# howird/humanoid

Measured on NVIDIA B200. Metric: env_steps_per_sec, higher is better.
Workload: dtype f32

## Files before the change

humanoid_b200/csrc/phc_kernels.cu:

```cuda
#include <algorithm>
#include <atomic>
#include <cfloat>
#include <cstdint>
#include <cstdio>
#include <cstdlib>
#include <cstring>
#include <new>

#include <cuda_bf16.h>
#include <cuda_runtime.h>

#include "../../include/phc_b200.h"
#include "phc_math.cuh"

namespace phc {

constexpr int J24 = PHC_NUM_BODIES;
constexpr int SELF_DIM = PHC_SELF_OBS_DIM;
constexpr int TASK_DIM = PHC_TASK_OBS_DIM;

static thread_local int g_last_cuda_error = 0;

static inline int cuda_fail(cudaError_t e) {
  g_last_cuda_error = (int)e;
// ... 889 lines not shown

constexpr int ROW13 = J24 * 13;
constexpr int FRAME_FLOATS = J24 * 13;
constexpr int FRAME_F4 = FRAME_FLOATS / 4;
constexpr int STAGE_FLOATS = SELF_DIM + TASK_DIM;

constexpr int EP_SUM_COLS = 12;

struct StepParams {
  LibDev L;
  PhcBodyState body;
  int16_t* progress;
  int16_t* progress_mirror;
  const float* start;
  const float* start_off;
  const float* goff;
  const int64_t* ids;
  const float* term_dist;
  uint32_t reset_mask;
  int use_mean, early, advance, T;
  float dt;
  PhcRewardSpec rwd;
  float* obs;
  int64_t obs_stride;
  float* rew;
  float* raw;
  int64_t raw_stride;
  uint8_t* reset;
  uint8_t* term;
  double* moments;
  int moment_buckets;
  int multi_prefetch;
  int moments_bulk;
  uint8_t *ep_terminals, *ep_truncations, *ep_masks;
  float* ep_returns;
  int32_t* ep_lengths;
  double* ep_sums;
  int ep_buckets, ep_raw_cols;
  float* mpjpe;
  float* obs_norm;
  int64_t obs_norm_stride;
  const float* norm_mean;
  const float* norm_var;
  float norm_eps, norm_clip;
  int norm_bf16;
  const float* dof_force;
  int64_t dof_force_stride;
  const float* dof_vel;
  int64_t dof_vel_stride, dof_vel_estride;
  float power_coef;
  int power_col;
  int64_t n;
  int first_wave_blocks;
  int spec_fault;
  unsigned long long* trace;
  const uint8_t* env_mask;
  int obs_only;
  int aos;
  int obs_vec2;
  float* rew_out;
  uint8_t* reset_out;
  uint8_t* term_out;
  float* ref_dof_pos;
  int64_t ref_dof_pos_stride;
  ObsFlags of;
  int selfw;
  int reset_on;
  ResetTargets rw;
  unsigned* tile_counter;
};

__host__ __device__ __forceinline__ bool default_obs_flags(const ObsFlags& f) { return f.hcol && f.local_root && f.upright; }

__device__ __forceinline__ void write_ref_dof_pos(const StepParams& p, int64_t env, int b, int64_t f0, int64_t f1, float bl) {
  if (b < 1) return;
  const Quat lr = quat_slerp(ld4v(p.L.lrs + (f0 * J24 + b) * 4), ld4v(p.L.lrs + (f1 * J24 + b) * 4), bl);
  st3(p.ref_dof_pos + env * p.ref_dof_pos_stride + (b - 1) * 3, quat_exp_map(lr));
}

__device__ __forceinline__ float norm_clamp(float y, float clip) { return y < -clip ? -clip : (y > clip ? clip : y); }
__device__ __forceinline__ void norm_column(const float* means, const float* vars, float eps, int64_t col, float& mean,
                                            float& sd, float& r) {
  mean = means[col];
  const float v = vars[col] + eps;
  sd = v >= FLT_MIN && v <= FLT_MAX ? sqrt_faithful(v) : sqrtf(v);
  r = rcp_approx(sd);
}
__device__ __forceinline__ void norm_column(const StepParams& p, int64_t col, float& mean, float& sd, float& r) {
  norm_column(p.norm_mean, p.norm_var, p.norm_eps, col, mean, sd, r);
}
__device__ __forceinline__ float norm_value(float x, float mean, float sd, float r, float clip) {
  const float a = x - mean;
  const float y = div_faithful(a, sd, r);
  return norm_clamp(y != y ? a * r : y, clip);
}

__device__ __forceinline__ float power_partial(const StepParams& p, int64_t env, int b) {
  if (b == 0) return 0.0f;
  const float* f = p.dof_force + env * p.dof_force_stride + (b - 1) * 3;
  const float* v = p.dof_vel + env * p.dof_vel_stride + (int64_t)(b - 1) * 3 * p.dof_vel_estride;
  return (fabsf(__ldcg(f) * __ldcg(v)) + fabsf(__ldcg(f + 1) * __ldcg(v + p.dof_vel_estride))) +
         fabsf(__ldcg(f + 2) * __ldcg(v + 2 * p.dof_vel_estride));
}
__device__ __forceinline__ float power_reward(const StepParams& p, const float* row24, int prog) {
  const float r = (-p.power_coef) * row_sum24(row24);
  return prog <= 3 ? 0.0f : r;
// ... 446 lines not shown
  static_assert(EPB * J24 == 96, "three warps, one role each");
  const int w = threadIdx.x >> 5, b = threadIdx.x & 31;
  const bool act = b < J24;
  const float len = S.meta_len[f], mdt = S.meta_mdt[f];
  const int nf = S.meta_nf[f];
  const int64_t st = S.meta_st[f];
  const float t = reset_start_time(p.rw, env, len);
  RefBody own;
  if (act) {
    int64_t f0, f1;
    float bl;
    reset_query_frames32(w == 1 ? 1 : 0, p.dt, t, len, nf, mdt, st, f0, f1, bl);
    if (w < 2) {
      const bool A = w == 0;
      own = blend_ref3(p.L.packed + f0 * FRAME_FLOATS, p.L.packed + f1 * FRAME_FLOATS, bl, A ? S.goff[f][0] : 0.0f,
                       A ? S.goff[f][1] : 0.0f, A ? S.goff[f][2] : 0.0f, b);
      if (A) {
        reset_store_body(p.rw, env, b, t, own.pos, own.rot, own.vel, own.ang, false);
        put13(S.sim + f * ROW13 + b * 13, own.pos, own.rot, own.vel, own.ang);
        if (b == 0) {
          if (p.progress_mirror) p.progress_mirror[env] = 0;
          const Heading h0 = heading_quat_inv(heading_source(own.rot, p.of.upright));
          S.nroot[f][0] = own.pos.x, S.nroot[f][1] = own.pos.y, S.nroot[f][2] = own.pos.z;
          S.nroot[f][3] = h0.z, S.nroot[f][4] = h0.w;
        }
      }
    } else {
      reset_store_dof(p.L, p.rw, env, b, f0, f1, bl);
      if (p.ref_dof_pos && b >= 1) {
        int64_t g0, g1;
        float gl;
        reset_query_frames32(1, p.dt, t, len, nf, mdt, st, g0, g1, gl);
        const Quat lr = quat_slerp(ld4v(p.L.lrs + (g0 * J24 + b) * 4), ld4v(p.L.lrs + (g1 * J24 + b) * 4), gl);
        st3(p.ref_dof_pos + env * p.ref_dof_pos_stride + (b - 1) * 3, quat_exp_map(lr));
      }
    }
  }
  __syncthreads();
  if (!act || w == 2) return;
  const int SW = DEF ? SELF_DIM : p.selfw;
  const Vec3 root_pos = {S.nroot[f][0], S.nroot[f][1], S.nroot[f][2]};
  const Heading hi = {S.nroot[f][3], S.nroot[f][4]};
  const HeadingRot hr = heading_rot(hi);
  float* row = S.frames + f * (SW + TASK_DIM);
  if (w == 0) {
    emit_self_obs<DEF>(row, p.of, b, root_pos, hi, hr, own.pos, own.rot, own.vel, own.ang);
  } else {
    const float* d = S.sim + f * ROW13 + b * 13;
    emit_task_obs<DEF>(row + SW, b, hi, hr, root_pos, Vec3{d[0], d[1], d[2]}, Quat{d[3], d[4], d[5], d[6]},
                       Vec3{d[7], d[8], d[9]}, Vec3{d[10], d[11], d[12]}, own);
  }
}

template <int EPB, int MINB, bool NORM = false, bool EP = false, bool RESET = false, bool DEF = true>
__global__ void __launch_bounds__(EPB* J24, MINB) step_fast_kernel(const __grid_constant__ StepParams p) {
  extern __shared__ __align__(16) unsigned char smem_raw[];
  FastSmem<EPB>& S = *reinterpret_cast<FastSmem<EPB>*>(smem_raw);
  constexpr int NT = EPB * J24;
  static_assert(4 * EPB <= 32, "reductions run on one warp");
  static_assert(!NORM || DEF, "the normaliser epilogue is laid out for the default 934-float rows");
  const int tid = threadIdx.x;
  const int64_t env0 = (int64_t)blockIdx.x * EPB;
  const int nvalid = p.n <= env0 ? 0 : (int)((p.n - env0) < EPB ? (p.n - env0) : EPB);
  PHC_STAMP(0);

  if (p.first_wave_blocks > 0) asm volatile("griddepcontrol.launch_dependents;\n" ::: "memory");
  const bool speculate = blockIdx.x < (unsigned)p.first_wave_blocks;
  if (tid < 32) {
    static_assert(EPB == 4, "phase 0 maps 8 lanes to each of 4 envs");
    if (tid == 0) mbar_init(&S.bar, 1);
    __syncwarp();
    const int le = tid >> 3, j = tid & 7;
    const bool act = le < nvalid;
    const bool lead = act && j == 0;
    const int64_t env = env0 + (act ? le : 0);
    const int adv = p.advance ? 1 : 0;
    float* fr = S.frames + le * (4 * FRAME_FLOATS);
    int64_t sid = -1, st = 0;
    int nf = 2, sprog = 0;
    float len = 1.0f, mdt = 1.0f, sstart = 0.0f, ssoff = 0.0f;
    int c_f0 = 0, c_f1 = 0;
    float c_bl = 0.0f, c_t = 0.0f;
    if (speculate && act && j < 3) {
      sid = p.ids[env];
      sprog = (int)p.progress[env];
      sstart = p.start[env];
      ssoff = p.start_off[env];
      if (p.spec_fault) {
        if (p.spec_fault & 1) sprog -= 1;
        if (p.spec_fault & 2) sstart += 1.0f / 30.0f;
        if (p.spec_fault & 4) sprog -= 2;
        if (p.spec_fault & 8) sid += 1;
      }
      const int64_t c = sid < 0 ? 0 : (sid >= p.L.M ? p.L.M - 1 : sid);
      len = p.L.len[c];
      nf = (int)p.L.nf[c];
      mdt = p.L.mdt[c];
      st = p.L.starts[c];
      c_t = (float)(int16_t)(sprog + adv + j) * p.dt + sstart + ssoff;
      calc_frame_blend32(c_t, len, nf, mdt, c_f0, c_f1, c_bl);
    }
    const int hi1 = __shfl_sync(0xffffffffu, c_f1, (tid & ~7) + 1);
    const int hi2 = __shfl_sync(0xffffffffu, c_f1, (tid & ~7) + 2);
    const int s_lo = c_f0;
    const bool all3 = hi2 - s_lo <= 3 && hi2 >= hi1;
    const int s_hi = all3 ? hi2 : hi1;
    const bool spec = speculate && lead && s_hi - s_lo <= 3 && s_hi >= s_lo;
    if (spec) {
      const uint32_t bytes = (uint32_t)(s_hi - s_lo + 1) * (uint32_t)(FRAME_FLOATS * 4);
      mbar_expect_tx(&S.bar, bytes);
      bulk_g2s(fr, p.L.packed + (st + s_lo) * FRAME_FLOATS, bytes, &S.bar);
    }
    const bool block_sim = p.body.pos.stride_env == ROW13;
    if (speculate && lead && (block_sim ? le == 0 : true)) {
      const uint32_t bytes = (block_sim ? (uint32_t)nvalid : 1u) * (uint32_t)(ROW13 * 4);
      asm volatile("cp.async.bulk.prefetch.L2.global [%0], %1;\n" ::"l"(p.body.pos.ptr + env * p.body.pos.stride_env),
                   "r"(bytes)
                   : "memory");
    }
    asm volatile("griddepcontrol.wait;\n" ::: "memory");
    if (p.first_wave_blocks <= 0) asm volatile("griddepcontrol.launch_dependents;\n" ::: "memory");
    PHC_STAMP(2);
    int prog_in = 0;
    bool ok = false;
    float start = 0.0f, soff = 0.0f, g0 = 0.0f, g1 = 0.0f, g2 = 0.0f;
    int64_t id = 0;
    if (lead) {
      prog_in = (int)__ldcg(p.progress + env);
      id = __ldcg(p.ids + env);
      start = __ldcg(p.start + env);
      soff = __ldcg(p.start_off + env);
      if (p.goff) {
        g0 = __ldcg(p.goff + env * 3 + 0);
        g1 = __ldcg(p.goff + env * 3 + 1);
        g2 = __ldcg(p.goff + env * 3 + 2);
      }
      if (block_sim ? le == 0 : true) {
        const uint32_t bytes = (block_sim ? (uint32_t)nvalid : 1u) * (uint32_t)(ROW13 * 4);
        mbar_expect_tx(&S.bar, bytes);
        bulk_g2s(S.sim + le * ROW13, p.body.pos.ptr + env * p.body.pos.stride_env, bytes, &S.bar);
      }
      const int dd = prog_in - sprog;
      ok = speculate && id == sid && __float_as_uint(start) == __float_as_uint(sstart) &&
           __float_as_uint(soff) == __float_as_uint(ssoff) && (dd == 0 || (dd == 1 && all3));
    }
    const int d = (prog_in - sprog) & 1;
    const int src0 = (tid & ~7) + d, src1 = src0 + 1;
    int a_f0 = __shfl_sync(0xffffffffu, c_f0, src0), a_f1 = __shfl_sync(0xffffffffu, c_f1, src0);
    int b_f0 = __shfl_sync(0xffffffffu, c_f0, src1), b_f1 = __shfl_sync(0xffffffffu, c_f1, src1);
    float a_bl = __shfl_sync(0xffffffffu, c_bl, src0), b_bl = __shfl_sync(0xffffffffu, c_bl, src1);
    float a_t = __shfl_sync(0xffffffffu, c_t, src0);
    const bool redo = lead && spec && !ok;
    const unsigned any_redo = __ballot_sync(0xffffffffu, redo);
    if (any_redo) {
      if (tid == 0) mbar_arrive(&S.bar);
      mbar_wait(&S.bar, 0);
    }
    if (lead) {
      int prog = prog_in;
      if (p.advance) prog = (int)(int16_t)(prog + 1);
      if (!ok) {
        len = p.L.len[id];
        nf = (int)p.L.nf[id];
        mdt = p.L.mdt[id];
        st = p.L.starts[id];
        a_t = (float)(int16_t)prog * p.dt + start + soff;
        calc_frame_blend32(a_t, len, nf, mdt, a_f0, a_f1, a_bl);
        const float t1 = (float)(int16_t)(prog + 1) * p.dt + start + soff;
        calc_frame_blend32(t1, len, nf, mdt, b_f0, b_f1, b_bl);
      }
      S.bl[0][le] = a_bl;
      S.bl[1][le] = b_bl;
      S.prog[le] = prog;
      S.pass[le] = a_t >= len;
      S.fallen[le] = 0;
      if (p.advance) {
        p.progress[env] = (int16_t)prog;
        if (p.progress_mirror) p.progress_mirror[env] = (int16_t)prog;
      }
      S.goff[le][0] = g0;
      S.goff[le][1] = g1;
      S.goff[le][2] = g2;
      if (RESET) {
        S.meta_len[le] = len, S.meta_mdt[le] = mdt, S.meta_nf[le] = nf, S.meta_st[le] = st;
      }
      if (p.ref_dof_pos) S.row1[0][le] = st + b_f0, S.row1[1][le] = st + b_f1;
      if (ok && spec) {
        S.slot[0][0][le] = a_f0 - s_lo;
        S.slot[0][1][le] = a_f1 - s_lo;
        S.slot[1][0][le] = b_f0 - s_lo;
        S.slot[1][1][le] = b_f1 - s_lo;
      } else {
        const float* tab = p.L.packed + st * FRAME_FLOATS;
        const int lo = a_f0 < b_f0 ? a_f0 : b_f0;
        int hi = a_f1 > b_f1 ? a_f1 : b_f1;
        hi = hi > a_f0 ? hi : a_f0;
        hi = hi > b_f0 ? hi : b_f0;
        if (hi - lo <= 3) {
          S.slot[0][0][le] = a_f0 - lo;
          S.slot[0][1][le] = a_f1 - lo;
          S.slot[1][0][le] = b_f0 - lo;
          S.slot[1][1][le] = b_f1 - lo;
          const uint32_t bytes = (uint32_t)(hi - lo + 1) * (uint32_t)(FRAME_FLOATS * 4);
          mbar_expect_tx(&S.bar, bytes);
          bulk_g2s(fr, tab + (int64_t)lo * FRAME_FLOATS, bytes, &S.bar);
        } else {
          S.slot[0][0][le] = 0;
          S.slot[0][1][le] = a_f1 - a_f0;
          S.slot[1][0][le] = 2;
          S.slot[1][1][le] = 2 + (b_f1 - b_f0);
          const uint32_t ba = (uint32_t)(a_f1 - a_f0 + 1) * (uint32_t)(FRAME_FLOATS * 4);
          const uint32_t bb = (uint32_t)(b_f1 - b_f0 + 1) * (uint32_t)(FRAME_FLOATS * 4);
          mbar_expect_tx(&S.bar, ba + bb);
          bulk_g2s(fr, tab + (int64_t)a_f0 * FRAME_FLOATS, ba, &S.bar);
          bulk_g2s(fr + 2 * FRAME_FLOATS, tab + (int64_t)b_f0 * FRAME_FLOATS, bb, &S.bar);
        }
      }
    }
    __syncwarp();
    if (tid == 0) {
      S.parity = any_redo ? 1 : 0;
      mbar_arrive(&S.bar);
    }
    PHC_STAMP(1);
  } else {
    asm volatile("griddepcontrol.wait;\n" ::: "memory");
    if (tid >= 32 && tid < 32 + nvalid) {
      const int le = tid - 32;
      const float* rq = p.body.pos.ptr + (env0 + le) * p.body.pos.stride_env + 3;
      const Quat rq4 = Quat{__ldcg(rq), __ldcg(rq + 1), __ldcg(rq + 2), __ldcg(rq + 3)};
      const Heading h0 = heading_quat_inv(DEF ? rq4 : heading_source(rq4, p.of.upright));
      S.hz[le] = h0.z;
      S.hw[le] = h0.w;
    }
  }
  __syncthreads();
  mbar_wait(&S.bar, (uint32_t)S.parity);
  PHC_STAMP(3);

  const int e = tid / J24, b = tid % J24;
  const bool valid = e < nvalid;
  Vec3 pos, vel, ang;
  Quat rot;
  RefBody r1;
  if (valid) {
    const float* d = S.sim + e * ROW13 + b * 13;
    pos = {d[0], d[1], d[2]};
    rot = {d[3], d[4], d[5], d[6]};
    vel = {d[7], d[8], d[9]};
    ang = {d[10], d[11], d[12]};
    const float* fr = S.frames + e * (4 * FRAME_FLOATS);
    {
      const RefBody r0 = blend_ref2(fr + S.slot[0][0][e] * FRAME_FLOATS, fr + S.slot[0][1][e] * FRAME_FLOATS,
                                    S.bl[0][e], S.goff[e], b);
      float sp, sr, sv, sa;
      reward_partials(pos, rot, vel, ang, r0, sp, sr, sv, sa);
      S.part[0][e][b] = sp;
      S.part[1][e][b] = sr;
      S.part[2][e][b] = sv;
      S.part[3][e][b] = sa;
      const float dist = norm3(pos - r0.pos);
      S.part[4][e][b] = dist;
      if (!p.use_mean && (p.reset_mask >> b & 1u) && dist > p.term_dist[b]) S.fallen[e] = 1;
      if (p.dof_force) S.part[5][e][b] = power_partial(p, env0 + e, b);
    }
    r1 = blend_ref2(fr + S.slot[1][0][e] * FRAME_FLOATS, fr + S.slot[1][1][e] * FRAME_FLOATS, S.bl[1][e], S.goff[e], b);
  }
  PHC_STAMP(4);
  __syncthreads();

  bool my_rst = false;
  int rst_mask = 0;
  if constexpr (RESET) {
    if (p.reset_on) {
      if (p.use_mean) {
        if (tid < nvalid) {
          float sel[J24];
          int m = 0;
#pragma unroll
          for (int j = 0; j < J24; ++j)
            if (p.reset_mask >> j & 1u) sel[m++] = S.part[4][tid][j];
          const int first = __ffs(p.reset_mask) - 1;
          bool fallen = p.early && m > 0 && (aten_row_sum(sel, m) / (float)m) > p.term_dist[first < 0 ? 0 : first];
          fallen = fallen && (S.prog[tid] > 1);
          S.rst[tid] = (S.pass[tid] || fallen) ? 1 : 0;
        }
        __syncthreads();
      }
#pragma unroll
      for (int i = 0; i < EPB; ++i) {
        int r = 0;
        if (i < nvalid) r = p.use_mean ? S.rst[i] : ((S.pass[i] || (p.early && S.fallen[i] && S.prog[i] > 1)) ? 1 : 0);
        rst_mask |= r << i;
        if (i == e) my_rst = valid && r;
      }
#pragma unroll
      for (int i = 0; i < EPB; ++i)
        if (rst_mask >> i & 1) reset_prefetch<EPB>(p, S, i, env0 + i);
    }
  }

  const int SW = DEF ? SELF_DIM : p.selfw;
  const int RW = SW + TASK_DIM;
  if (valid && !(RESET && my_rst)) {
    const Vec3 root_pos = {S.sim[e * ROW13 + 0], S.sim[e * ROW13 + 1], S.sim[e * ROW13 + 2]};
    const Heading hi = {S.hz[e], S.hw[e]};
    const HeadingRot hr = heading_rot(hi);
    float* row = S.frames + e * RW;
    emit_self_obs<DEF>(row, p.of, b, root_pos, hi, hr, pos, rot, vel, ang);
    emit_task_obs<DEF>(row + SW, b, hi, hr, root_pos, pos, rot, vel, ang, r1);
  }
  if constexpr (RESET) {
    if (rst_mask) {
#pragma unroll 1
      for (int i = 0; i < EPB; ++i)
        if (rst_mask >> i & 1) reset_in_step<EPB, DEF>(p, S, i, env0 + i);
    }
  }
  fence_proxy_async();
  PHC_STAMP(5);
  __syncthreads();
  PHC_STAMP(6);

  const uint32_t out_bytes = (uint32_t)nvalid * (uint32_t)(RW * 4);
  const bool bulk_ok = (out_bytes & 15u) == 0;
  if (bulk_ok) {
    if (tid == NT - 1 && out_bytes) bulk_s2g(p.obs + env0 * RW, S.frames, out_bytes);
  } else if (DEF || ((nvalid * RW) & 1) == 0) {
    float2* dst = reinterpret_cast<float2*>(p.obs + env0 * RW);
    const float2* src = reinterpret_cast<const float2*>(S.frames);
    for (int i = tid; i < nvalid * RW / 2; i += NT) dst[i] = src[i];
  } else {
    for (int i = tid; i < nvalid * RW; i += NT) p.obs[env0 * RW + i] = S.frames[i];
  }
  if (p.moments) {
    double* mom = p.moments + (int64_t)(blockIdx.x % p.moment_buckets) * 2 * RW;
    if (p.moments_bulk) {
      constexpr int CH = 624;
      static_assert(CH * 8 <= (int)sizeof(S.sim) && CH * 8 <= (int)sizeof(S.frames) - EPB * STAGE_FLOATS * 4, "regions");
      double* regA = reinterpret_cast<double*>(S.sim);
      double* regB = reinterpret_cast<double*>(S.frames + EPB * RW);
      const int total = 2 * RW;
      for (int c0 = 0, r = 0; c0 < total; c0 += CH, ++r) {
        double* reg = (r & 1) ? regB : regA;
        const int cnt = total - c0 < CH ? total - c0 : CH;
        if (r >= 2) {
          if (tid == 0) bulk_wait_read_all_but_one();
          __syncthreads();
        }
        for (int i = tid; i < cnt; i += NT) {
          const int g = c0 + i;
          const bool sq = g >= RW;
          const int col = sq ? g - RW : g;
          double acc = 0.0;
          for (int ee = 0; ee < nvalid; ++ee) {
            const double x = (double)S.frames[ee * RW + col];
            acc += sq ? x * x : x;
          }
          reg[i] = acc;
        }
        fence_proxy_async();
        __syncthreads();
        if (tid == 0) bulk_reduce_add_f64(mom + c0, reg, (uint32_t)cnt * 8u);
      }
      if (NORM && p.obs_norm) {
        if (tid == 0) bulk_wait_read();
        __syncthreads();
      }
    } else {
      for (int c = tid; c < RW; c += NT) {
        double s1 = 0.0, s2 = 0.0;
        for (int ee = 0; ee < nvalid; ++ee) {
          const double x = (double)S.frames[ee * RW + c];
          s1 += x;
          s2 += x * x;
        }
        atomicAdd(mom + c, s1);
        atomicAdd(mom + RW + c, s2);
      }
    }
  }
  if (p.ref_dof_pos && valid && !(RESET && my_rst))
    write_ref_dof_pos(p, env0 + e, b, S.row1[0][e], S.row1[1][e], S.bl[1][e]);
  const bool norm_inplace = NORM && p.obs_norm && bulk_ok && !p.norm_bf16;
  if (norm_inplace) {
    if (tid == NT - 1) bulk_wait_read();
    __syncthreads();
    float2* st = reinterpret_cast<float2*>(S.frames);
    for (int c2 = tid; c2 < STAGE_FLOATS / 2; c2 += NT) {
      float m0, sd0, r0, m1, sd1, r1;
      norm_column(p, 2 * c2, m0, sd0, r0);
      norm_column(p, 2 * c2 + 1, m1, sd1, r1);
      for (int ee = 0; ee < nvalid; ++ee) {
        const float2 x = st[ee * (STAGE_FLOATS / 2) + c2];
        st[ee * (STAGE_FLOATS / 2) + c2] =
            make_float2(norm_value(x.x, m0, sd0, r0, p.norm_clip), norm_value(x.y, m1, sd1, r1, p.norm_clip));
      }
    }
    fence_proxy_async();
    __syncthreads();
    if (tid == NT - 1) bulk_s2g(p.obs_norm + env0 * STAGE_FLOATS, S.frames, out_bytes);
  }
  constexpr int NORM16_SPLIT = 932;
  static_assert(EPB != 4 || (NORM16_SPLIT * 4 <= (int)sizeof(S.sim) && (EPB * STAGE_FLOATS / 2 - NORM16_SPLIT) * 4 <=
                                 (int)sizeof(S.frames) - EPB * STAGE_FLOATS * 4), "bf16 staging fits the dead regions");
  const bool norm16_staged =
      NORM && p.obs_norm && bulk_ok && p.norm_bf16 && nvalid == EPB && EPB == 4 && ((uintptr_t)p.obs_norm & 15) == 0;
  if (norm16_staged) {
    __nv_bfloat162* pa = reinterpret_cast<__nv_bfloat162*>(S.sim);
    __nv_bfloat162* pb = reinterpret_cast<__nv_bfloat162*>(S.frames + EPB * STAGE_FLOATS);
    const float2* src = reinterpret_cast<const float2*>(S.frames);
    for (int c2 = tid; c2 < STAGE_FLOATS / 2; c2 += NT) {
      float m0, sd0, r0, m1, sd1, r1;
      norm_column(p, 2 * c2, m0, sd0, r0);
      norm_column(p, 2 * c2 + 1, m1, sd1, r1);
#pragma unroll
      for (int ee = 0; ee < EPB; ++ee) {
        const int i = ee * (STAGE_FLOATS / 2) + c2;
        const float2 x = src[i];
        const __nv_bfloat162 y = __floats2bfloat162_rn(norm_value(x.x, m0, sd0, r0, p.norm_clip),
                                                       norm_value(x.y, m1, sd1, r1, p.norm_clip));
        if (i < NORM16_SPLIT) pa[i] = y;
        else pb[i - NORM16_SPLIT] = y;
      }
    }
    fence_proxy_async();
    __syncthreads();
    if (tid == NT - 1) {
      __nv_bfloat162* dst = reinterpret_cast<__nv_bfloat162*>(p.obs_norm) + env0 * (STAGE_FLOATS / 2);
      bulk_s2g(dst, pa, NORM16_SPLIT * 4);
      bulk_s2g(dst + NORM16_SPLIT, pb, (EPB * STAGE_FLOATS / 2 - NORM16_SPLIT) * 4);
    }
  }
  if (tid < 32) {
    const int le = tid >> 2, k = tid & 3;
    const bool act = le < nvalid && tid < 4 * EPB;
    float term_k = 0.0f;
    float ep_ret = 0.0f;
    int32_t ep_len = 0;
    if constexpr (EP) {
      if (p.ep_returns && act && k == 0) {
        ep_ret = p.ep_returns[env0 + le];
        ep_len = p.ep_lengths[env0 + le];
      }
    }
    if (act) {
      const float kk = k == 0 ? p.rwd.k_pos : k == 1 ? p.rwd.k_rot : k == 2 ? p.rwd.k_vel : p.rwd.k_ang_vel;
      term_k = expf((-kk) * (row_sum24(&S.part[k][le][0]) / 24.0f));
      p.raw[(env0 + le) * p.raw_stride + k] = term_k;
    }
    const int base = tid & ~3;
    const float t0 = __shfl_sync(0xffffffffu, term_k, base), t1 = __shfl_sync(0xffffffffu, term_k, base + 1);
    const float t2 = __shfl_sync(0xffffffffu, term_k, base + 2), t3 = __shfl_sync(0xffffffffu, term_k, base + 3);
    float r = 0.0f, pr = 0.0f;
    int flags = 0;
    if (act && k == 0) {
      r = p.rwd.w_pos * t0 + p.rwd.w_rot * t1 + p.rwd.w_vel * t2 + p.rwd.w_ang_vel * t3;
      if (p.dof_force) {
        pr = power_reward(p, &S.part[5][le][0], S.prog[le]);
        r += pr;
        p.raw[(env0 + le) * p.raw_stride + p.power_col] = pr;
      }
      p.rew[env0 + le] = r;
      if (p.rew_out) p.rew_out[env0 + le] = r;
    }
    if (act && k == 1) {
      bool fallen = false;
      if (p.early) {
        if (p.use_mean) {
          float sel[J24];
          int m = 0;
#pragma unroll
          for (int j = 0; j < J24; ++j)
            if (p.reset_mask >> j & 1u) sel[m++] = S.part[4][le][j];
          const int first = __ffs(p.reset_mask) - 1;
          fallen = m > 0 && (aten_row_sum(sel, m) / (float)m) > p.term_dist[first < 0 ? 0 : first];
        } else {
          fallen = S.fallen[le] != 0;
        }
        fallen = fallen && (S.prog[le] > 1);
      }
      const bool rs = S.pass[le] || fallen;
      const bool cleared = RESET && p.reset_on;
      p.term[env0 + le] = (fallen && !cleared) ? 1 : 0;
      p.reset[env0 + le] = (rs && !cleared) ? 1 : 0;
      if (p.term_out) p.term_out[env0 + le] = fallen ? 1 : 0;
      if (p.reset_out) p.reset_out[env0 + le] = rs ? 1 : 0;
      flags = (rs ? 1 : 0) | (fallen ? 2 : 0);
    }
    if (act && k == 2 && p.mpjpe) p.mpjpe[env0 + le] = row_sum24(&S.part[4][le][0]) / 24.0f;
    if constexpr (EP) if (p.ep_returns) {
      flags = __shfl_sync(0xffffffffu, flags, base + 1);
      float v[EP_SUM_COLS];
#pragma unroll
      for (int i = 0; i < EP_SUM_COLS; ++i) v[i] = 0.0f;
      if (act && k == 0) {
        const int64_t e = env0 + le;
        const bool rs = flags & 1, tm = (flags & 2) != 0, tr = rs && !tm;
        p.ep_terminals[e] = tm ? 1 : 0;
        p.ep_truncations[e] = tr ? 1 : 0;
        p.ep_masks[e] = tr ? 0 : 1;
        float ret = ep_ret;
        int32_t len = ep_len;
        if (rs) {
          v[0] = 1.0f;
          v[1] = ret;
          v[2] = (float)len;
          v[3] = tr ? 1.0f : 0.0f;
          ret = 0.0f;
          len = 0;
        }
        p.ep_returns[e] = ret + r;
        p.ep_lengths[e] = len + 1;
        v[4] = t0, v[5] = t1, v[6] = t2, v[7] = t3;
        if (p.dof_force) {
#pragma unroll
          for (int i = 8; i < EP_SUM_COLS; ++i)
            if (i == 4 + p.power_col) v[i] = pr;
        }
      }
      float mine = 0.0f;
#pragma unroll
      for (int i = 0; i < EP_SUM_COLS; ++i) {
        v[i] += __shfl_xor_sync(0xffffffffu, v[i], 4);
        v[i] += __shfl_xor_sync(0xffffffffu, v[i], 8);
        const float tot = __shfl_sync(0xffffffffu, v[i], 0);
        if (tid == i) mine = tot;
      }
      if (tid < 4 + p.ep_raw_cols && mine != 0.0f)
        atomicAdd(p.ep_sums + (int64_t)(blockIdx.x % p.ep_buckets) * EP_SUM_COLS + tid, (double)mine);
    }
  }

  if (NORM && p.obs_norm && !norm_inplace && !norm16_staged) {
    float2* dst = reinterpret_cast<float2*>(p.obs_norm + env0 * STAGE_FLOATS);
    __nv_bfloat162* dst16 = reinterpret_cast<__nv_bfloat162*>(p.obs_norm) + env0 * (STAGE_FLOATS / 2);
    const float2* src = reinterpret_cast<const float2*>(S.frames);
    for (int c2 = tid; c2 < STAGE_FLOATS / 2; c2 += NT) {
      float m0, sd0, r0, m1, sd1, r1;
      norm_column(p, 2 * c2, m0, sd0, r0);
      norm_column(p, 2 * c2 + 1, m1, sd1, r1);
      for (int ee = 0; ee < nvalid; ++ee) {
        const float2 x = src[ee * (STAGE_FLOATS / 2) + c2];
        const float y0 = norm_value(x.x, m0, sd0, r0, p.norm_clip), y1 = norm_value(x.y, m1, sd1, r1, p.norm_clip);
        if (p.norm_bf16) dst16[ee * (STAGE_FLOATS / 2) + c2] = __floats2bfloat162_rn(y0, y1);
        else dst[ee * (STAGE_FLOATS / 2) + c2] = make_float2(y0, y1);
      }
    }
  }
  if (bulk_ok && tid == NT - 1) bulk_wait_read();
  if (p.moments && p.moments_bulk && tid == 0) bulk_wait_read();
  PHC_STAMP(7);
}

constexpr int PS_STAGES = 2;
constexpr int PS_EPB = 4;
constexpr int PS_CONSUMERS = PS_EPB * J24;
constexpr int PS_THREADS = PS_CONSUMERS + 32;

template <int SLOTS>
struct PersistStage {
  float sim[PS_EPB * ROW13];
  float frames[PS_EPB * SLOTS * FRAME_FLOATS];
  float part[6][PS_EPB][J24];
  float bl[2][PS_EPB];
  int slot[2][2][PS_EPB];
  int64_t far[PS_EPB];
  float goff[PS_EPB][4];
  float hz[PS_EPB], hw[PS_EPB];
  int prog[PS_EPB], pass[PS_EPB], fallen[PS_EPB];
  int tile;
  int pad_[3];
  static_assert(SLOTS * FRAME_FLOATS >= STAGE_FLOATS, "the obs stage aliases the frame buffer");
};
template <int SLOTS>
struct PersistSmem {
  PersistStage<SLOTS> st[PS_STAGES];
  unsigned long long full[PS_STAGES], empty[PS_STAGES];
};
static_assert(sizeof(PersistStage<3>) % 16 == 0 && sizeof(PersistStage<4>) % 16 == 0,
              "stages keep the 16-byte alignment of the TMA destinations");

__device__ __forceinline__ void consumer_sync() { asm volatile("bar.sync 1, %0;" ::"r"(PS_CONSUMERS) : "memory"); }

template <int SLOTS, int BLOCKS_PER_SM, bool MOM = false>
__global__ void __launch_bounds__(PS_THREADS, BLOCKS_PER_SM) step_persist_kernel(const __grid_constant__ StepParams p) {
  extern __shared__ __align__(16) unsigned char smem_raw[];
  PersistSmem<SLOTS>& M = *reinterpret_cast<PersistSmem<SLOTS>*>(smem_raw);
  using Stage = PersistStage<SLOTS>;
  const int tid = threadIdx.x;
  const int num_tiles = (int)((p.n + PS_EPB - 1) / PS_EPB);
  if (tid == 0) {
#pragma unroll
    for (int s = 0; s < PS_STAGES; ++s) {
      mbar_init(&M.full[s], 1);
      mbar_init(&M.empty[s], MOM ? PS_CONSUMERS / 32 : 1);
    }
  }
  __syncthreads();

  if (tid >= PS_CONSUMERS) {
    const int lane = tid - PS_CONSUMERS;
    const int le = lane >> 3, j = lane & 7;
    asm volatile("griddepcontrol.launch_dependents;\n" ::: "memory");
// ... 1468 lines not shown
  p.raw_stride = a->reward_raw_stride;
  p.reset = a->reset_buf;
  p.term = a->terminate_buf;
  p.moments = a->obs_moments;
  p.moment_buckets = a->obs_moments_buckets > 1 ? a->obs_moments_buckets : 1;
  p.moments_bulk = 0;
  {
    static int mp = -1;
    if (mp < 0) {
      const char* w = getenv("PHC_MULTI_PREFETCH");
      mp = (w && w[0] == '0') ? 0 : 1;
    }
    p.multi_prefetch = mp;
  }
  p.ep_terminals = a->ep_terminals;
  p.ep_truncations = a->ep_truncations;
  p.ep_masks = a->ep_masks;
  p.ep_returns = a->ep_returns;
  p.ep_lengths = a->ep_lengths;
  p.ep_sums = a->ep_sums;
  p.ep_buckets = a->ep_buckets;
  p.ep_raw_cols = a->ep_raw_cols;
  if (a->ep_returns) {
    if (!a->ep_terminals || !a->ep_truncations || !a->ep_masks || !a->ep_lengths || !a->ep_sums) return PHC_ERR_NULL;
    if (a->ep_buckets < 1 || a->ep_buckets > 4096 || a->ep_raw_cols < 0 || a->ep_raw_cols > EP_SUM_COLS - 4) return PHC_ERR_SHAPE;
  }
  if (a->obs_moments_buckets < 0 || a->obs_moments_buckets > 4096) return PHC_ERR_SHAPE;
  p.mpjpe = a->mpjpe;
  p.obs_norm = a->obs_norm;
  p.obs_norm_stride = a->obs_norm_stride;
  p.norm_mean = a->norm_mean;
  p.norm_var = a->norm_var;
  p.norm_eps = a->norm_epsilon;
  p.norm_clip = a->norm_clip;
  p.norm_bf16 = (a->flags & PHC_STEP_OBS_NORM_BF16) ? 1 : 0;
  if (a->obs_norm) {
    if (!a->norm_mean || !a->norm_var) return PHC_ERR_NULL;
    if (a->obs_norm_stride < W || !(a->norm_clip > 0.0f)) return PHC_ERR_SHAPE;
  }
  p.dof_force = a->dof_force;
  p.dof_force_stride = a->dof_force_stride;
  p.dof_vel = a->dof_vel;
  p.dof_vel_stride = a->dof_vel_stride;
  p.dof_vel_estride = a->dof_vel_elem_stride;
  p.power_coef = a->rew_power_coef;
  p.power_col = a->power_col;
  if (a->dof_force) {
    if (!a->dof_vel) return PHC_ERR_NULL;
    if (a->power_col < 4 || a->power_col >= a->reward_raw_stride || a->dof_force_stride < 69 ||
        a->dof_vel_elem_stride < 1)
      return PHC_ERR_SHAPE;
  }
  p.first_wave_blocks = 0;
  p.spec_fault = g_spec_fault;
  p.env_mask = nullptr;
  p.obs_only = 0;
  {
    const int64_t nw = (n + 3) / 4 * 3;
    if (g_trace && (g_trace_launch + 1) * nw <= g_trace_capacity) {
      p.trace = g_trace + g_trace_launch * nw * 8;
      ++g_trace_launch;
    } else {
      p.trace = nullptr;
    }
  }
  p.n = n;
  const PhcBodyState& s = a->body;
  p.aos = s.rot.ptr == s.pos.ptr + 3 && s.vel.ptr == s.pos.ptr + 7 && s.ang_vel.ptr == s.pos.ptr + 10 &&
          s.pos.stride_body == 13 && s.rot.stride_body == 13 && s.vel.stride_body == 13 &&
          s.ang_vel.stride_body == 13 && s.rot.stride_env == s.pos.stride_env &&
          s.vel.stride_env == s.pos.stride_env && s.ang_vel.stride_env == s.pos.stride_env &&
          ((uintptr_t)s.pos.ptr & 15) == 0 && (s.pos.stride_env % 4) == 0 && s.pos.stride_env >= ROW13;
  p.obs_vec2 = ((uintptr_t)a->obs_buf & 7) == 0 && (a->obs_stride % 2) == 0;
  return PHC_OK;
}

static int g_force_generic = -1;
static int g_fast_epb = -1;
static int g_pdl = -1;

static void init_options() {
  if (g_force_generic < 0) {
    const char* v = getenv("PHC_STEP_GENERIC");
    g_force_generic = (v && v[0] == '1') ? 1 : 0;
  }
  if (g_fast_epb < 0) {
    const char* w = getenv("PHC_STEP_EPB");
    g_fast_epb = (w && w[0] == '8') ? 8 : 4;
  }
  if (g_pdl < 0) {
    const char* w = getenv("PHC_STEP_PDL");
    g_pdl = (w && w[0] == '0') ? 0 : 1;
  }
  if (g_moments_bulk < 0) {
    const char* w = getenv("PHC_MOMENTS_BULK");
    g_moments_bulk = (w && w[0] == '1') ? 1 : 0;
  }
  if (g_persist < 0) {
    const char* w = getenv("PHC_STEP_PERSIST");
    g_persist = (w && w[0] >= '0' && w[0] <= '3') ? w[0] - '0' : 1;
    g_persist_pdl = g_pdl;
    const char* m = getenv("PHC_STEP_PERSIST_MIN");
    if (m && atoll(m) > 0) g_persist_min = atoll(m);
  }
}

// ... 83 lines not shown
                                     ((uintptr_t)p.obs_norm & (p.norm_bf16 ? 3 : 15)) == 0));
  static bool attr_gen[64] = {};
  static int first_wave[64] = {};
  static bool attr_persist[3][64] = {};
  static int sm_count[64] = {};
  const bool persist = fast && def && g_persist != 0 &&
                       (g_persist >= 2 || p.n >= (p.moments ? g_persist_min_moments : g_persist_min)) && !p.obs_norm &&
                       !p.ep_returns && !p.reset_on && !p.ref_dof_pos && !p.trace && lib->tile_counters &&
                       !(args->flags & PHC_STEP_MAPPED_HOST_IO);
  if (persist) {
    if (!sm_count[dev]) PHC_CUDA(cudaDeviceGetAttribute(&sm_count[dev], cudaDevAttrMultiProcessorCount, dev));
    const bool mom = p.moments != nullptr;
    const bool four = !mom && g_persist == 3;
    const int which = mom ? 2 : four ? 1 : 0;
    auto kern = mom ? step_persist_kernel<3, 4, true> : four ? step_persist_kernel<4, 4> : step_persist_kernel<3, 5>;
    const size_t smem = four ? sizeof(PersistSmem<4>) : sizeof(PersistSmem<3>);
    if (!attr_persist[which][dev]) {
      PHC_CUDA(cudaFuncSetAttribute(kern, cudaFuncAttributeMaxDynamicSharedMemorySize, (int)smem));
      attr_persist[which][dev] = true;
    }
    if (lib->unspeculated_steps > 0) --lib->unspeculated_steps;
    p.tile_counter = lib->tile_counters + 2 * (lib->tile_seq.fetch_add(1u, std::memory_order_relaxed) % TILE_SLOTS);
    const int64_t tiles = (p.n + PS_EPB - 1) / PS_EPB;
    const int64_t resident = (int64_t)sm_count[dev] * (four || mom ? 4 : 5);
    cudaLaunchConfig_t cfg{};
    cfg.gridDim = dim3((unsigned)(tiles < resident ? tiles : resident));
    cfg.blockDim = dim3(PS_THREADS);
    cfg.dynamicSmemBytes = smem;
    cfg.stream = stream;
    cudaLaunchAttribute at[1];
    at[0].id = cudaLaunchAttributeProgrammaticStreamSerialization;
    at[0].val.programmaticStreamSerializationAllowed = 1;
    cfg.attrs = at;
    cfg.numAttrs = g_persist_pdl ? 1 : 0;
    PHC_CUDA(cudaLaunchKernelEx(&cfg, kern, p));
    return launch_status();
  }
  bool reset_after = false;
  if (fast) {
    if (!first_wave[dev]) {
      int sms = 0, per_sm = 0;
      PHC_CUDA(cudaDeviceGetAttribute(&sms, cudaDevAttrMultiProcessorCount, dev));
      PHC_CUDA(cudaFuncSetAttribute(step_fast_kernel<4, 8>, cudaFuncAttributeMaxDynamicSharedMemorySize,
                                    (int)sizeof(FastSmem<4>)));
      PHC_CUDA(cudaOccupancyMaxActiveBlocksPerMultiprocessor(&per_sm, step_fast_kernel<4, 8>, 4 * J24,
                                                             sizeof(FastSmem<4>)));
      first_wave[dev] = sms * (per_sm > 0 ? per_sm : 1);
    }
    p.first_wave_blocks = (g_pdl && !(args->flags & PHC_STEP_MAPPED_HOST_IO)) ? first_wave[dev] : 0;
    if (lib->unspeculated_steps > 0) {
      p.first_wave_blocks = 0;
      --lib->unspeculated_steps;
    }
    static bool attr[7][64] = {};
    const bool pdl = g_pdl != 0;
    constexpr size_t SM = sizeof(FastSmem<4>);
    p.moments_bulk = (p.moments && g_moments_bulk && ((uintptr_t)p.moments & 15) == 0) ? 1 : 0;
    const bool in_kernel = p.reset_on && p.rw.state_init <= PHC_STATE_INIT_RANDOM;
    reset_after = p.reset_on && !in_kernel;
    StepParams pk = p;
    if (reset_after) pk.reset_on = 0;
    if (!def) rc = launch_step(step_fast_kernel<4, 8, false, true, true, false>, SM, 4, pk, stream, &attr[6][dev], pdl);
    else if (in_kernel) {
      if (p.obs_norm) rc = launch_step(step_fast_kernel<4, 8, true, true, true>, SM, 4, pk, stream, &attr[5][dev], pdl);
      else rc = launch_step(step_fast_kernel<4, 8, false, true, true>, SM, 4, pk, stream, &attr[4][dev], pdl);
    } else if (p.obs_norm && p.ep_returns)
      rc = launch_step(step_fast_kernel<4, 8, true, true>, SM, 4, pk, stream, &attr[3][dev], pdl);
    else if (p.ep_returns) rc = launch_step(step_fast_kernel<4, 8, false, true>, SM, 4, pk, stream, &attr[2][dev], pdl);
    else if (p.obs_norm) rc = launch_step(step_fast_kernel<4, 8, true>, SM, 4, pk, stream, &attr[1][dev], pdl);
    else rc = launch_step(step_fast_kernel<4, 8>, SM, 4, pk, stream, &attr[0][dev], pdl);
    if (rc != PHC_OK || !reset_after) return rc;
  } else {
  const bool multi = !g_force_generic && p.T > 1 && p.aos && p.L.packed && p.obs_vec2 && !p.obs_norm && def &&
                     !(args->flags & PHC_STEP_MAPPED_HOST_IO);
  static bool attr_multi[64] = {}, attr_multi2[64] = {};
  const int multi_groups = g_multi_groups ? g_multi_groups : 2;
  if (multi && multi_groups == 2) {
    if (!attr_multi2[dev]) {
      PHC_CUDA(cudaFuncSetAttribute(step_multi2_kernel, cudaFuncAttributeMaxDynamicSharedMemorySize, (int)sizeof(Multi2Smem)));
      attr_multi2[dev] = true;
    }
    step_multi2_kernel<<<(unsigned)((p.n + MULTI_EPB - 1) / MULTI_EPB), 2 * MULTI_EPB * J24, sizeof(Multi2Smem), stream>>>(p);
    rc = launch_status();
  } else if (multi) {
    rc = launch_step(step_multi_kernel, sizeof(MultiSmem), MULTI_EPB, p, stream, &attr_multi[dev], false);
  } else {
    rc = launch_step(step_kernel<STEP_EPB>, sizeof(StepSmem<STEP_EPB>), STEP_EPB, p, stream, &attr_gen[dev], false);
  }
  if (rc == PHC_OK && p.ep_returns) {
    episode_bucket_kernel<<<(unsigned)((p.n + 255) / 256), 256, 0, stream>>>(p);
    rc = launch_status();
  }
  reset_after = p.reset_on != 0;
  }
  if (rc == PHC_OK && reset_after) {
    ResetParams r;
    rc = reset_fill(lib, args->auto_reset, n, r);
    if (rc) return rc;
    r.mask = p.reset;
    r.norm = NormOut{p.obs_norm, p.obs_norm_stride, p.norm_mean, p.norm_var, p.norm_eps, p.norm_clip, p.norm_bf16};
    r.moments = p.moments;
    r.moment_buckets = p.moment_buckets;
    r.moments_mode = p.moments ? 2 : 0;
    rc = reset_launch(r, stream);
  }
  return rc;
}

bool lib_has_dof_state(const PhcLib* lib) { return lib && lib->d.lrs && lib->d.dvs; }

extern "C" {

int phc_step_fused(const PhcLib* lib, const PhcStepArgs* args, int64_t n, phc_stream_t stream) {
  return step_fused_mirrored(lib, args, n, stream, nullptr);
}

int phc_obs_moments(const float* x, int64_t rows, int64_t cols, int64_t row_stride, double* sums,
                    phc_stream_t stream) {
  if (rows == 0 || cols == 0) return PHC_OK;
  if (rows < 0 || cols < 0 || row_stride < cols) return PHC_ERR_SHAPE;
  if (!x || !sums) return PHC_ERR_NULL;
  int64_t rpb = MOM_ROWS_PER_BLOCK;
// ... 163 lines not shown
```

profiles/trace_step.py:

```python
import os
import sys

sys.path.insert(0, os.path.dirname(os.path.dirname(os.path.abspath(__file__))))
import numpy as np
import torch

from humanoid_b200 import HumanoidPHC, MotionLib, _cabi, synth

N = int(sys.argv[1]) if len(sys.argv) > 1 else 4096
dev = torch.device("cuda", 0)
lib_data = synth.make_motion_lib(N, 60, 300, (30,), seed=1234, device=dev)
lib = MotionLib(lib_data, device=dev)
clock = synth.make_clock(lib_data, N, seed=1235, max_progress=30)
envs = []
for r in range(17):
    ref = lib.get_motion_state(clock.sampled_motion_ids, synth.reward_time(clock, extra_steps=r + 1), clock.global_offset)
    env = HumanoidPHC(lib, N, device=dev)
    env.set_sim_state(synth.make_sim_state(ref, seed=1236 + r), copy=False)
    env.set_clock(clock)
    envs.append(env)
for i in range(20):
    envs[i % 17].post_physics_step(True)
torch.cuda.synchronize()
nw = (N + 3) // 4 * 3
# ... 2 lines not shown
capi = _cabi.load()
for e in envs:
    e._step_args = None
    e.post_physics_step(True)
torch.cuda.synchronize()
capi.phc_set_trace_buffer(buf.data_ptr(), K * nw)
graph = torch.cuda.CUDAGraph()
stream = torch.cuda.Stream()
stream.wait_stream(torch.cuda.current_stream())
with torch.cuda.stream(stream):
    with torch.cuda.graph(graph, stream=stream):
        for k in range(K):
            envs[k].post_physics_step(True)
capi.phc_set_trace_buffer(None, 0)
torch.cuda.synchronize()
graph.replay()
torch.cuda.synchronize()
buf.zero_()
graph.replay()
torch.cuda.synchronize()
T = [b.cpu().numpy().reshape(-1, 3, 8).astype(np.float64) for b in buf.view(K, -1)]
names = ["entry", "tma issued", "dep wait done", "data landed", "phase1 done", "stage written", "past bar3", "exit"]
t00 = T[0][:, :, 0].min()
prev_end = None
for k, t in enumerate(T):
    t = (t - t00) / 1e3
    w0 = t[:, 0, :]
    first, last = t[:, :, 0].min(), t[:, :, 7].max()
    line = f"kernel {k}: first entry {first:7.2f}  last exit {last:7.2f}  span {last - first:5.2f} us"
    if prev_end is not None:
        line += f"  | starts {first - prev_end:+.2f} us vs previous kernel's last exit; period {last - prev_last:5.2f} us"
    print(line)
    if k >= K - 2:
        for j in (0, 2, 1, 3, 4, 5, 6, 7):
            col = w0[:, j] - (prev_end if prev_end is not None else first)
            print(f"    warp0 {names[j]:14s} (rel. prev exit): min {col.min():6.2f}  median {np.median(col):6.2f}  "
                  f"p90 {np.percentile(col, 90):6.2f}  max {col.max():6.2f}")
    prev_end, prev_last = last, last

t = (T[-1] - t00) / 1e3
w0 = t[:, 0, :]
last_prev = ((T[-2] - t00) / 1e3)[:, :, 7].max()
exit_rel = t[:, :, 7].max(axis=1) - last_prev
post = w0[:, 1] - w0[:, 2]
land = w0[:, 3] - w0[:, 1]
entry_rel = w0[:, 0] - last_prev
print("\nlatest-exiting blocks of the last kernel (us relative to the previous kernel's last exit):")
for i in np.argsort(-exit_rel)[:10]:
    print(f"  block {i:5d}: entry {entry_rel[i]:6.2f}  wait->issued {post[i]:5.2f}  issued->landed {land[i]:5.2f}  "
          f"phase1 {w0[i, 4] - w0[i, 3]:5.2f}  phase2 {w0[i, 5] - w0[i, 4]:5.2f}  exit {exit_rel[i]:5.2f}")
for name, arr in (("wait->issued", post), ("issued->landed", land), ("exit", exit_rel)):
    qs = np.percentile(arr, [50, 90, 99, 100])
    print(f"  {name:15s}: p50 {qs[0]:5.2f}  p90 {qs[1]:5.2f}  p99 {qs[2]:5.2f}  max {qs[3]:5.2f}")
```

Baseline: 584.7 million.

## Add plain step kernel variant and limit four-row speculative prefetch to subset of blocks

Adds a PLAIN template instantiation of the fast step kernel that compiles out optional epilogues (dof force, ref dof pos, moments, mirrors, mpjpe, rew_out, use_mean) when none are requested. It also limits the speculative four-frame TMA prefetch to a subset of first-wave blocks (spec4_blocks). Other blocks prefetch three rows and issue a follow-up bulk copy for the extra row only when progress actually advanced. This aims to cut speculative bytes and per-thread branching, at the cost of an extra dependent copy on some blocks. A trace code is also recorded for profiling.

Result: faster. 603.9 million, median of 6 (+3.3%).

```diff
diff --git a/humanoid_b200/csrc/phc_kernels.cu b/humanoid_b200/csrc/phc_kernels.cu
--- a/humanoid_b200/csrc/phc_kernels.cu
+++ b/humanoid_b200/csrc/phc_kernels.cu
@@ -965,6 +965,7 @@
   int power_col;
   int64_t n;
   int first_wave_blocks;
+  int spec4_blocks;
   int spec_fault;
   unsigned long long* trace;
   const uint8_t* env_mask;
@@ -1517,13 +1518,18 @@
   }
 }
 
-template <int EPB, int MINB, bool NORM = false, bool EP = false, bool RESET = false, bool DEF = true>
+template <int EPB, int MINB, bool NORM = false, bool EP = false, bool RESET = false, bool DEF = true, bool PLAIN = false>
 __global__ void __launch_bounds__(EPB* J24, MINB) step_fast_kernel(const __grid_constant__ StepParams p) {
   extern __shared__ __align__(16) unsigned char smem_raw[];
   FastSmem<EPB>& S = *reinterpret_cast<FastSmem<EPB>*>(smem_raw);
   constexpr int NT = EPB * J24;
   static_assert(4 * EPB <= 32, "reductions run on one warp");
   static_assert(!NORM || DEF, "the normaliser epilogue is laid out for the default 934-float rows");
+  static_assert(!PLAIN || (!NORM && !EP && !RESET && DEF), "the plain step carries none of the epilogues");
+  const bool use_mean = !PLAIN && p.use_mean;
+  const bool dof_force = !PLAIN && p.dof_force;
+  const bool ref_dof_pos = !PLAIN && p.ref_dof_pos;
+  const bool moments = !PLAIN && p.moments;
   const int tid = threadIdx.x;
   const int64_t env0 = (int64_t)blockIdx.x * EPB;
   const int nvalid = p.n <= env0 ? 0 : (int)((p.n - env0) < EPB ? (p.n - env0) : EPB);
@@ -1531,6 +1537,7 @@
 
   if (p.first_wave_blocks > 0) asm volatile("griddepcontrol.launch_dependents;\n" ::: "memory");
   const bool speculate = blockIdx.x < (unsigned)p.first_wave_blocks;
+  const bool spec4 = blockIdx.x < (unsigned)p.spec4_blocks;
   if (tid < 32) {
     static_assert(EPB == 4, "phase 0 maps 8 lanes to each of 4 envs");
     if (tid == 0) mbar_init(&S.bar, 1);
@@ -1569,7 +1576,7 @@
     const int hi2 = __shfl_sync(0xffffffffu, c_f1, (tid & ~7) + 2);
     const int s_lo = c_f0;
     const bool all3 = hi2 - s_lo <= 3 && hi2 >= hi1;
-    const int s_hi = all3 ? hi2 : hi1;
+    const int s_hi = all3 && spec4 ? hi2 : hi1;
     const bool spec = speculate && lead && s_hi - s_lo <= 3 && s_hi >= s_lo;
     if (spec) {
       const uint32_t bytes = (uint32_t)(s_hi - s_lo + 1) * (uint32_t)(FRAME_FLOATS * 4);
@@ -1586,7 +1593,7 @@
     asm volatile("griddepcontrol.wait;\n" ::: "memory");
     if (p.first_wave_blocks <= 0) asm volatile("griddepcontrol.launch_dependents;\n" ::: "memory");
     PHC_STAMP(2);
-    int prog_in = 0;
+    int prog_in = 0, dd = 0;
     bool ok = false;
     float start = 0.0f, soff = 0.0f, g0 = 0.0f, g1 = 0.0f, g2 = 0.0f;
     int64_t id = 0;
@@ -1595,7 +1602,7 @@
       id = __ldcg(p.ids + env);
       start = __ldcg(p.start + env);
       soff = __ldcg(p.start_off + env);
-      if (p.goff) {
+      if (PLAIN || p.goff) {
         g0 = __ldcg(p.goff + env * 3 + 0);
         g1 = __ldcg(p.goff + env * 3 + 1);
         g2 = __ldcg(p.goff + env * 3 + 2);
@@ -1605,7 +1612,7 @@
         mbar_expect_tx(&S.bar, bytes);
         bulk_g2s(S.sim + le * ROW13, p.body.pos.ptr + env * p.body.pos.stride_env, bytes, &S.bar);
       }
-      const int dd = prog_in - sprog;
+      dd = prog_in - sprog;
       ok = speculate && id == sid && __float_as_uint(start) == __float_as_uint(sstart) &&
            __float_as_uint(soff) == __float_as_uint(ssoff) && (dd == 0 || (dd == 1 && all3));
     }
@@ -1641,7 +1648,7 @@
       S.fallen[le] = 0;
       if (p.advance) {
         p.progress[env] = (int16_t)prog;
-        if (p.progress_mirror) p.progress_mirror[env] = (int16_t)prog;
+        if (!PLAIN && p.progress_mirror) p.progress_mirror[env] = (int16_t)prog;
       }
       S.goff[le][0] = g0;
       S.goff[le][1] = g1;
@@ -1649,12 +1656,17 @@
       if (RESET) {
         S.meta_len[le] = len, S.meta_mdt[le] = mdt, S.meta_nf[le] = nf, S.meta_st[le] = st;
       }
-      if (p.ref_dof_pos) S.row1[0][le] = st + b_f0, S.row1[1][le] = st + b_f1;
+      if (ref_dof_pos) S.row1[0][le] = st + b_f0, S.row1[1][le] = st + b_f1;
       if (ok && spec) {
         S.slot[0][0][le] = a_f0 - s_lo;
         S.slot[0][1][le] = a_f1 - s_lo;
         S.slot[1][0][le] = b_f0 - s_lo;
         S.slot[1][1][le] = b_f1 - s_lo;
+        if (dd == 1 && s_hi < hi2) {
+          const uint32_t bytes = (uint32_t)(hi2 - s_hi) * (uint32_t)(FRAME_FLOATS * 4);
+          mbar_expect_tx(&S.bar, bytes);
+          bulk_g2s(fr + (s_hi - s_lo + 1) * FRAME_FLOATS, p.L.packed + (st + s_hi + 1) * FRAME_FLOATS, bytes, &S.bar);
+        }
       } else {
         const float* tab = p.L.packed + st * FRAME_FLOATS;
         const int lo = a_f0 < b_f0 ? a_f0 : b_f0;
@@ -1683,6 +1695,13 @@
       }
     }
     __syncwarp();
+    if (p.trace) {
+      const unsigned fetch = __ballot_sync(0xffffffffu, lead && ok && spec && dd == 1 && s_hi < hi2);
+      const unsigned fresh = __ballot_sync(0xffffffffu, lead && !spec);
+      if (tid == 0)
+        p.trace[((size_t)blockIdx.x * 3 + 1) * 8 + 1] =
+            16u | (spec4 ? 1u : 0u) | (fetch ? 2u : 0u) | (any_redo ? 4u : 0u) | (fresh ? 8u : 0u);
+    }
     if (tid == 0) {
       S.parity = any_redo ? 1 : 0;
       mbar_arrive(&S.bar);
@@ -1726,8 +1745,8 @@
       S.part[3][e][b] = sa;
       const float dist = norm3(pos - r0.pos);
       S.part[4][e][b] = dist;
-      if (!p.use_mean && (p.reset_mask >> b & 1u) && dist > p.term_dist[b]) S.fallen[e] = 1;
-      if (p.dof_force) S.part[5][e][b] = power_partial(p, env0 + e, b);
+      if (!use_mean && (p.reset_mask >> b & 1u) && dist > p.term_dist[b]) S.fallen[e] = 1;
+      if (dof_force) S.part[5][e][b] = power_partial(p, env0 + e, b);
     }
     r1 = blend_ref2(fr + S.slot[1][0][e] * FRAME_FLOATS, fr + S.slot[1][1][e] * FRAME_FLOATS, S.bl[1][e], S.goff[e], b);
   }
@@ -1798,7 +1817,7 @@
   } else {
     for (int i = tid; i < nvalid * RW; i += NT) p.obs[env0 * RW + i] = S.frames[i];
   }
-  if (p.moments) {
+  if (moments) {
     double* mom = p.moments + (int64_t)(blockIdx.x % p.moment_buckets) * 2 * RW;
     if (p.moments_bulk) {
       constexpr int CH = 624;
@@ -1845,7 +1864,7 @@
       }
     }
   }
-  if (p.ref_dof_pos && valid && !(RESET && my_rst))
+  if (ref_dof_pos && valid && !(RESET && my_rst))
     write_ref_dof_pos(p, env0 + e, b, S.row1[0][e], S.row1[1][e], S.bl[1][e]);
   const bool norm_inplace = NORM && p.obs_norm && bulk_ok && !p.norm_bf16;
   if (norm_inplace) {
@@ -1921,18 +1940,18 @@
     int flags = 0;
     if (act && k == 0) {
       r = p.rwd.w_pos * t0 + p.rwd.w_rot * t1 + p.rwd.w_vel * t2 + p.rwd.w_ang_vel * t3;
-      if (p.dof_force) {
+      if (dof_force) {
         pr = power_reward(p, &S.part[5][le][0], S.prog[le]);
         r += pr;
         p.raw[(env0 + le) * p.raw_stride + p.power_col] = pr;
       }
       p.rew[env0 + le] = r;
-      if (p.rew_out) p.rew_out[env0 + le] = r;
+      if (!PLAIN && p.rew_out) p.rew_out[env0 + le] = r;
     }
     if (act && k == 1) {
       bool fallen = false;
       if (p.early) {
-        if (p.use_mean) {
+        if (use_mean) {
           float sel[J24];
           int m = 0;
 #pragma unroll
@@ -1953,7 +1972,7 @@
       if (p.reset_out) p.reset_out[env0 + le] = rs ? 1 : 0;
       flags = (rs ? 1 : 0) | (fallen ? 2 : 0);
     }
-    if (act && k == 2 && p.mpjpe) p.mpjpe[env0 + le] = row_sum24(&S.part[4][le][0]) / 24.0f;
+    if (!PLAIN && act && k == 2 && p.mpjpe) p.mpjpe[env0 + le] = row_sum24(&S.part[4][le][0]) / 24.0f;
     if constexpr (EP) if (p.ep_returns) {
       flags = __shfl_sync(0xffffffffu, flags, base + 1);
       float v[EP_SUM_COLS];
@@ -2014,7 +2033,7 @@
     }
   }
   if (bulk_ok && tid == NT - 1) bulk_wait_read();
-  if (p.moments && p.moments_bulk && tid == 0) bulk_wait_read();
+  if (moments && p.moments_bulk && tid == 0) bulk_wait_read();
   PHC_STAMP(7);
 }
 
@@ -3589,6 +3608,7 @@
       return PHC_ERR_SHAPE;
   }
   p.first_wave_blocks = 0;
+  p.spec4_blocks = 0;
   p.spec_fault = g_spec_fault;
   p.env_mask = nullptr;
   p.obs_only = 0;
@@ -3778,7 +3798,11 @@
       p.first_wave_blocks = 0;
       --lib->unspeculated_steps;
     }
-    static bool attr[7][64] = {};
+    const int64_t grid = (p.n + 3) / 4;
+    p.spec4_blocks = p.first_wave_blocks > grid ? (int)(p.first_wave_blocks - grid) : 0;
+    const bool plain = !p.dof_force && !p.ref_dof_pos && !p.mpjpe && !p.use_mean && !p.moments && !p.rew_out &&
+                       !p.progress_mirror && p.goff;
+    static bool attr[8][64] = {};
     const bool pdl = g_pdl != 0;
     constexpr size_t SM = sizeof(FastSmem<4>);
     p.moments_bulk = (p.moments && g_moments_bulk && ((uintptr_t)p.moments & 15) == 0) ? 1 : 0;
@@ -3794,6 +3818,8 @@
       rc = launch_step(step_fast_kernel<4, 8, true, true>, SM, 4, pk, stream, &attr[3][dev], pdl);
     else if (p.ep_returns) rc = launch_step(step_fast_kernel<4, 8, false, true>, SM, 4, pk, stream, &attr[2][dev], pdl);
     else if (p.obs_norm) rc = launch_step(step_fast_kernel<4, 8, true>, SM, 4, pk, stream, &attr[1][dev], pdl);
+    else if (plain)
+      rc = launch_step(step_fast_kernel<4, 8, false, false, false, true, true>, SM, 4, pk, stream, &attr[7][dev], pdl);
     else rc = launch_step(step_fast_kernel<4, 8>, SM, 4, pk, stream, &attr[0][dev], pdl);
     if (rc != PHC_OK || !reset_after) return rc;
   } else {
diff --git a/profiles/trace_step.py b/profiles/trace_step.py
--- a/profiles/trace_step.py
+++ b/profiles/trace_step.py
@@ -78,3 +78,18 @@
 for name, arr in (("wait->issued", post), ("issued->landed", land), ("exit", exit_rel)):
     qs = np.percentile(arr, [50, 90, 99, 100])
     print(f"  {name:15s}: p50 {qs[0]:5.2f}  p90 {qs[1]:5.2f}  p99 {qs[2]:5.2f}  max {qs[3]:5.2f}")
+
+code = T[-1][:, 1, 1].astype(np.int64)
+if (code & 16).all():
+    redo = (code & 4) != 0
+    fetch = ((code & 2) != 0) & ~redo
+    fresh = ((code & 8) != 0) & ~redo & ~fetch
+    hit = ~redo & ~fetch & ~fresh
+    spec4 = (code & 1) != 0
+    print(f"\nphase-0 paths of the last kernel's {len(code)} blocks ({int(spec4.sum())} below spec4_blocks): "
+          f"four-row hit {int((hit & spec4).sum())}, three-row hit {int((hit & ~spec4).sum())}, "
+          f"extra-row fetch {int(fetch.sum())}, redo {int(redo.sum())}, no speculation {int(fresh.sum())}")
+    for name, sel in (("four-row hit", hit & spec4), ("three-row hit", hit & ~spec4), ("extra-row fetch", fetch)):
+        if sel.any():
+            print(f"  {name:15s}: median entry {np.median(entry_rel[sel]):6.2f}  issued->landed {np.median(land[sel]):5.2f}"
+                  f"  exit {np.median(exit_rel[sel]):5.2f}")
```
